# VisionDepth/VisionDepth3D

Hardware: AMD Instinct MI355X
Metric: stereo-pairs/sec end-to-end (depth+warp+fill+mux) (higher is better)
Workload: dtype f32; 1 GPU; 4k-dav2b-dibr; frame=3840x2160, format=Half-SBS, depth_model=depth-anything-v2-base, depth_net_dtype=float32 (the reference's precision), pixel_overlap=True, pixel_streams=2, clip_frames_all_ranks=32, params=render_cli.py defaults + dof_strength 2.0, dense DOF order (parity mode)

## Files before the change

### visiondepth3d_amd/csrc/vd3d_attn.hip

```cpp
#include "vd3d_dev.h"
#include "vd3d_kernels.h"
#include "vd3d_x3.h"

#include <mutex>

#define AT_D 64
#define AT_BQ 256
#define AT_BK 64
#define AT_NT 512
#define AT_NTERM(MODE) ((MODE) == 0 ? 3 : 2)
#define AT_TILE(MODE) (4 * AT_NTERM(MODE) * 2 * 64 * 16)
#define AT_STAGE(MODE) (2 * AT_TILE(MODE))
#define AT_NSTAGE 3
#define AT_LDS(MODE) (AT_NSTAGE * AT_STAGE(MODE))
#define AT_QBLK(MODE) (4 * AT_NTERM(MODE) * 2 * 32)
#define AT_QKV_SCALE 16.0f
#define AT_P_SCALE 1024.0f
#define AT_OP 272

struct vd_at_args {
  int B, H, T;
  int nq32, nkv, nqb;
  float c;
};

template <int MODE>
__global__ __launch_bounds__(256) void k_attn_x3_prep(const float* __restrict__ qkv, vd_at_args a, uint4* __restrict__ Qimg, uint4* __restrict__ Kimg,
                                                      uint4* __restrict__ Vimg) {
  constexpr int NTERM = AT_NTERM(MODE);
  const int which = blockIdx.z, bh = blockIdx.y, b = bh / a.H, h = bh - b * a.H;
  const int t_id = blockIdx.x * 256 + threadIdx.x;
  const size_t tok_stride = (size_t)3 * a.H * AT_D;
  float v[8];
  uint4* dst;
  if (which < 2) {
    const int rows = which == 0 ? a.nq32 * 32 : a.nkv * 64;
    const int t = t_id >> 3, c = t_id & 7;
    if (t >= rows) return;
    if (t < a.T) {
      const float* src = qkv + ((size_t)b * a.T + t) * tok_stride + (size_t)which * a.H * AT_D + h * AT_D + c * 8;
      const float4 lo = *reinterpret_cast<const float4*>(src), hi = *reinterpret_cast<const float4*>(src + 4);
      v[0] = lo.x; v[1] = lo.y; v[2] = lo.z; v[3] = lo.w; v[4] = hi.x; v[5] = hi.y; v[6] = hi.z; v[7] = hi.w;
    } else {
#pragma unroll
      for (int e = 0; e < 8; ++e) v[e] = 0.f;
    }
    const int ks = c >> 1, kh = c & 1;
    if (which == 0) dst = Qimg + ((size_t)bh * a.nq32 + (t >> 5)) * AT_QBLK(MODE) + (size_t)((ks * NTERM) * 2 + kh) * 32 + (t & 31);
    else dst = Kimg + ((size_t)bh * a.nkv + (t >> 6)) * (AT_TILE(MODE) / 16) + (size_t)((ks * NTERM) * 2 + kh) * 64 + (t & 63);
    x3_s8 o[NTERM];
    x3_split8_m<MODE>(v, AT_QKV_SCALE, o);
    const int ts = which == 0 ? 2 * 32 : 2 * 64;
#pragma unroll
    for (int t3 = 0; t3 < NTERM; ++t3) dst[(size_t)t3 * ts] = __builtin_bit_cast(uint4, o[t3]);
  } else {
    const int d = t_id & 63, kh = (t_id >> 6) & 1, ks = (t_id >> 7) & 3, tile = t_id >> 9;
    if (tile >= a.nkv) return;
    const int m = ks >> 1, j = ks & 1;
#pragma unroll
    for (int e = 0; e < 8; ++e) {
      const int kv = tile * 64 + 32 * m + (e & 3) + 8 * (2 * j + (e >> 2)) + 4 * kh;
      v[e] = kv < a.T ? qkv[((size_t)b * a.T + kv) * tok_stride + (size_t)2 * a.H * AT_D + h * AT_D + d] : 0.f;
    }
    x3_s8 o[NTERM];
    x3_split8_m<MODE>(v, AT_QKV_SCALE, o);
    dst = Vimg + ((size_t)bh * a.nkv + tile) * (AT_TILE(MODE) / 16) + (size_t)((ks * NTERM) * 2 + kh) * 64 + d;
#pragma unroll
    for (int t3 = 0; t3 < NTERM; ++t3) dst[(size_t)t3 * 128] = __builtin_bit_cast(uint4, o[t3]);
  }
}

#define AT_MM1(ACC0, AF0, ACC1, AF1, BF, ta, tb)                                               \
  ACC0 = x3_mfma<MODE>(AF0[ta], BF[tb], ACC0);                                                 \
  ACC1 = x3_mfma<MODE>(AF1[ta], BF[tb], ACC1);
#define AT_MM6(ACC0, AF0, ACC1, AF1, BF)                                                       \
  if (MODE == 0) { AT_MM1(ACC0, AF0, ACC1, AF1, BF, NTERM - 1, 0) AT_MM1(ACC0, AF0, ACC1, AF1, BF, 1, 1) AT_MM1(ACC0, AF0, ACC1, AF1, BF, 0, NTERM - 1) }                               \
  AT_MM1(ACC0, AF0, ACC1, AF1, BF, 1, 0) AT_MM1(ACC0, AF0, ACC1, AF1, BF, 0, 1) AT_MM1(ACC0, AF0, ACC1, AF1, BF, 0, 0)

template <int MODE>
__global__ __launch_bounds__(AT_NT) void k_attn_bf16x3(const uint4* __restrict__ Qimg, const uint4* __restrict__ Kimg, const uint4* __restrict__ Vimg,
                                                       float* __restrict__ out, vd_at_args a) {
  constexpr int NTERM = AT_NTERM(MODE), TILE = AT_TILE(MODE), STAGE = AT_STAGE(MODE), NP = TILE / (AT_NT * 16);
  extern __shared__ __attribute__((aligned(16))) uint8_t at_lds[];
  int bh, qb;
  {
    const int wg = blockIdx.x, x = wg & 7, idx = wg >> 3;
    const int g = idx / a.nqb;
    qb = idx - g * a.nqb;
    bh = g * 8 + x;
    if (bh >= a.B * a.H) return;
  }
  const int tid = threadIdx.x, lane = tid & 63, wave = __builtin_amdgcn_readfirstlane(tid >> 6);
  const int li = lane & 31, kh = lane >> 5;
  const int q0 = qb * AT_BQ + wave * 32;
  const int wave_base = (tid & ~63) * 16;

  x3_s8 qf[4][NTERM];
  {
    const int blk = min(q0 >> 5, a.nq32 - 1);
    const uint4* qp = Qimg + ((size_t)bh * a.nq32 + blk) * AT_QBLK(MODE) + kh * 32 + li;
#pragma unroll
    for (int ks = 0; ks < 4; ++ks)
#pragma unroll
      for (int t = 0; t < NTERM; ++t) qf[ks][t] = __builtin_bit_cast(x3_s8, qp[(ks * NTERM + t) * 64]);
  }
  const uint4* kimg = Kimg + (size_t)bh * a.nkv * (TILE / 16) + tid;
  const uint4* vimg = Vimg + (size_t)bh * a.nkv * (TILE / 16) + tid;
  auto dma = [&](int tile, int buf, int piece) {
    const int op = piece / 3, pp = piece - 3 * op;
    if (pp >= NP) return;
    const uint4* src = (op == 0 ? kimg : vimg) + (size_t)tile * (TILE / 16) + pp * AT_NT;
    uint8_t* dst = at_lds + buf * STAGE + op * TILE + pp * (AT_NT * 16) + wave_base;
    __builtin_amdgcn_global_load_lds((x3_glb_vp)src, (x3_lds_vp)dst, 16, 0, 0);
  };

  x3_f16 oacc[2];
#pragma unroll
  for (int dm = 0; dm < 2; ++dm)
#pragma unroll
    for (int r = 0; r < 16; ++r) oacc[dm][r] = 0.f;
  float m_run = -INFINITY, l_half = 0.f;

  const int last_tile = a.nkv - 1;
  auto tile_c = [&](int t) { return t < last_tile ? t : last_tile; };
#pragma unroll
  for (int p = 0; p < 6; ++p) dma(0, 0, p);
#pragma unroll
  for (int p = 0; p < 3; ++p) dma(tile_c(1), 1, p);
#pragma unroll
  for (int p = 3; p < 6; ++p) dma(tile_c(1), 1, p);
#pragma unroll
  for (int p = 0; p < 3; ++p) dma(tile_c(2), 2, p);
  if (NP == 3) asm volatile("s_waitcnt vmcnt(6)" ::: "memory"); else asm volatile("s_waitcnt vmcnt(4)" ::: "memory");
  __builtin_amdgcn_s_barrier();

  const int frag_off = (kh * 64 + li) * 16;
  auto st_step = [&](const uint8_t* sk, int ks, x3_f16 (&sa)[2]) {
    x3_s8 kf[2][NTERM];
#pragma unroll
    for (int m = 0; m < 2; ++m)
#pragma unroll
      for (int t = 0; t < NTERM; ++t) kf[m][t] = *reinterpret_cast<const x3_s8*>(sk + frag_off + ((ks * NTERM + t) * 2) * 1024 + m * 512);
    AT_MM6(sa[0], kf[0], sa[1], kf[1], qf[ks])
  };
#define AT_CHUNK_HINT(n)                                           \
  __builtin_amdgcn_sched_group_barrier(0x100, 6, 0);               \
  _Pragma("unroll") for (int i_ = 0; i_ < 12; ++i_) {              \
    __builtin_amdgcn_sched_group_barrier(0x008, 1, 0);             \
    __builtin_amdgcn_sched_group_barrier(0x002, n, 0);             \
  }                                                                \
  __builtin_amdgcn_sched_barrier(0);

  x3_f16 sacc[2];
#pragma unroll
  for (int m = 0; m < 2; ++m)
#pragma unroll
    for (int r = 0; r < 16; ++r) sacc[m][r] = 0.f;
#pragma unroll
  for (int ks = 0; ks < 4; ++ks) st_step(at_lds, ks, sacc);
  asm volatile("s_waitcnt lgkmcnt(0)" ::: "memory");
  __builtin_amdgcn_s_barrier();

  int cur = 0;
  for (int it = 0; it < a.nkv; ++it) {
    const int s1 = cur == 2 ? 0 : cur + 1, s2 = cur >= 1 ? cur - 1 : 2;
    const uint8_t* sk1 = at_lds + s1 * STAGE;
    const uint8_t* sv = at_lds + cur * STAGE + TILE;
    float z[2][16];
#pragma unroll
    for (int m = 0; m < 2; ++m)
#pragma unroll
      for (int r = 0; r < 16; ++r) z[m][r] = sacc[m][r] * a.c;
    if ((it + 1) * AT_BK > a.T) {
#pragma unroll
      for (int m = 0; m < 2; ++m)
#pragma unroll
        for (int r = 0; r < 16; ++r)
          if (it * AT_BK + 32 * m + (r & 3) + 8 * (r >> 2) + 4 * kh >= a.T) z[m][r] = -INFINITY;
    }
    x3_f16 sn[2];
#pragma unroll
    for (int m = 0; m < 2; ++m)
#pragma unroll
      for (int r = 0; r < 16; ++r) sn[m][r] = 0.f;
    dma(tile_c(it + 3), cur, 0);
    __builtin_amdgcn_sched_barrier(0);
    st_step(sk1, 0, sn);
    float mx = -INFINITY;
#pragma unroll
    for (int m = 0; m < 2; ++m)
#pragma unroll
      for (int r = 0; r < 16; ++r) mx = fmaxf(mx, z[m][r]);
    mx = fmaxf(mx, __shfl_xor(mx, 32, 64));
    const float m_new = fmaxf(m_run, mx);
    const float alpha = __builtin_amdgcn_exp2f(m_run - m_new);
    m_run = m_new;
    AT_CHUNK_HINT(2)
    float ps = 0.f;
#pragma unroll
    for (int m = 0; m < 2; ++m) {
      dma(tile_c(it + 3), cur, 1 + m);
      __builtin_amdgcn_sched_barrier(0);
      st_step(sk1, 1 + m, sn);
#pragma unroll
      for (int r = 0; r < 16; ++r) { z[m][r] = __builtin_amdgcn_exp2f(z[m][r] - m_new); ps += z[m][r]; }
      AT_CHUNK_HINT(4)
    }
    dma(tile_c(it + 2), s2, 3);
    __builtin_amdgcn_sched_barrier(0);
    st_step(sk1, 3, sn);
    l_half = l_half * alpha + ps;
#pragma unroll
    for (int dm = 0; dm < 2; ++dm)
#pragma unroll
      for (int r = 0; r < 16; ++r) oacc[dm][r] *= alpha;
    x3_s8 pf[2][NTERM];
    x3_split8_m<MODE>(&z[0][0], AT_P_SCALE, pf[0]);
    AT_CHUNK_HINT(7)
#pragma unroll
    for (int ks = 0; ks < 4; ++ks) {
      if (ks < 2) { dma(tile_c(it + 2), s2, 4 + ks); __builtin_amdgcn_sched_barrier(0); }
      if (ks < 3) x3_split8_m<MODE>(&z[(ks + 1) >> 1][8 * ((ks + 1) & 1)], AT_P_SCALE, pf[(ks + 1) & 1]);
      x3_s8 vf[2][NTERM];
#pragma unroll
      for (int dm = 0; dm < 2; ++dm)
#pragma unroll
        for (int t = 0; t < NTERM; ++t) vf[dm][t] = *reinterpret_cast<const x3_s8*>(sv + frag_off + ((ks * NTERM + t) * 2) * 1024 + dm * 512);
      AT_MM6(oacc[0], vf[0], oacc[1], vf[1], pf[ks & 1])
      AT_CHUNK_HINT(4)
    }
    if (NP == 3) asm volatile("s_waitcnt vmcnt(6) lgkmcnt(0)" ::: "memory"); else asm volatile("s_waitcnt vmcnt(4) lgkmcnt(0)" ::: "memory");
    __builtin_amdgcn_s_barrier();
#pragma unroll
    for (int m = 0; m < 2; ++m) sacc[m] = sn[m];
    cur = s1;
  }
#undef AT_CHUNK_HINT
  asm volatile("s_waitcnt vmcnt(0)" ::: "memory");
  __builtin_amdgcn_s_barrier();

  const float l_tot = l_half + __shfl_xor(l_half, 32, 64);
  const float inv = MODE == 1 ? 1.0f / (l_tot * (AT_P_SCALE * AT_QKV_SCALE)) : 1.0f / l_tot;
  uint8_t* ow = at_lds + wave * (32 * AT_OP);
#pragma unroll
  for (int dm = 0; dm < 2; ++dm)
#pragma unroll
    for (int g = 0; g < 4; ++g) {
      const float4 v4 = {oacc[dm][4 * g] * inv, oacc[dm][4 * g + 1] * inv, oacc[dm][4 * g + 2] * inv, oacc[dm][4 * g + 3] * inv};
      *reinterpret_cast<float4*>(ow + li * AT_OP + (32 * dm + 8 * g + 4 * kh) * 4) = v4;
    }
  asm volatile("s_waitcnt lgkmcnt(0)" ::: "memory");
  const int b = bh / a.H, h = bh - b * a.H;
#pragma unroll
  for (int i = 0; i < 8; ++i) {
    const int row = i * 4 + (lane >> 4), c4 = lane & 15;
    const int q = q0 + row;
    const float4 v4 = *reinterpret_cast<const float4*>(ow + row * AT_OP + c4 * 16);
    if (q < a.T) *reinterpret_cast<float4*>(out + (((size_t)b * a.T + q) * a.H + h) * AT_D + c4 * 4) = v4;
  }
}

#define AF_TILE (AT_BK * AT_D * 4)
#define AF_STAGE (2 * AF_TILE)
#define AF_LDS(NS) ((NS) * AF_STAGE)
static_assert(2 * AF_LDS(2) <= 160 * 1024, "two 4-wave workgroups per CU");
VD_DEV void af_st(const uint8_t* __restrict__ sk, const float (&qf)[32], int li, int kh, x3_f16 (&s)[2]) {
  const int kswz = (li & 15) << 4;
#pragma unroll
  for (int m = 0; m < 2; ++m)
#pragma unroll
    for (int r = 0; r < 16; ++r) s[m][r] = 0.f;
#pragma unroll
  for (int g = 0; g < 8; ++g) {
    float4 kf[2];
#pragma unroll
    for (int m = 0; m < 2; ++m) kf[m] = *reinterpret_cast<const float4*>(sk + (32 * m + li) * 256 + (((8 * kh + g) << 4) ^ kswz));
#pragma unroll
    for (int m = 0; m < 2; ++m) s[m] = __builtin_amdgcn_mfma_f32_32x32x2f32(kf[m].x, qf[4 * g], s[m], 0, 0, 0);
#pragma unroll
    for (int m = 0; m < 2; ++m) s[m] = __builtin_amdgcn_mfma_f32_32x32x2f32(kf[m].y, qf[4 * g + 1], s[m], 0, 0, 0);
#pragma unroll
    for (int m = 0; m < 2; ++m) s[m] = __builtin_amdgcn_mfma_f32_32x32x2f32(kf[m].z, qf[4 * g + 2], s[m], 0, 0, 0);
#pragma unroll
    for (int m = 0; m < 2; ++m) s[m] = __builtin_amdgcn_mfma_f32_32x32x2f32(kf[m].w, qf[4 * g + 3], s[m], 0, 0, 0);
  }
}
VD_DEV void af_pv(const uint8_t* __restrict__ sv, const x3_f16 (&p)[2], int li, int kh, x3_f16 (&oacc)[2]) {
#pragma unroll
  for (int m = 0; m < 2; ++m)
#pragma unroll
    for (int r = 0; r < 16; ++r) {
      const float2 vv = *reinterpret_cast<const float2*>(sv + (32 * m + (r & 3) + 8 * (r >> 2) + 4 * kh) * 256 + li * 8);
      oacc[0] = __builtin_amdgcn_mfma_f32_32x32x2f32(vv.x, p[m][r], oacc[0], 0, 0, 0);
      oacc[1] = __builtin_amdgcn_mfma_f32_32x32x2f32(vv.y, p[m][r], oacc[1], 0, 0, 0);
    }
}

template <int NW, int NS>
__global__ __launch_bounds__(NW * 64, NW == 4 ? 2 : 1) void k_attn_f32(const float* __restrict__ qkv, float* __restrict__ out, vd_at_args a) {
  static_assert((NW == 8 && NS == 3) || (NW == 4 && NS == 2), "built forms");
  constexpr int NP = 16 / NW;
  extern __shared__ __attribute__((aligned(16))) uint8_t at_lds[];
  int bh, qb;
  {
    const int wg = blockIdx.x, x = wg & 7, idx = wg >> 3;
    const int g = idx / a.nqb;
    qb = idx - g * a.nqb;
    bh = g * 8 + x;
    if (bh >= a.B * a.H) return;
  }
  const int tid = threadIdx.x, lane = tid & 63, wave = __builtin_amdgcn_readfirstlane(tid >> 6);
  const int li = lane & 31, kh = lane >> 5;
  const int q0 = qb * (NW * 32) + wave * 32;
  const bool live = NW == 8 || q0 < a.T;
  const int b = bh / a.H, h = bh - b * a.H;
  const size_t tok_stride = (size_t)3 * a.H * AT_D;
  const float* base = qkv + (size_t)b * a.T * tok_stride + h * AT_D;

  const int drow = tid >> 4, dpos = tid & 15, kchunk = dpos ^ (drow & 15);
  auto dma = [&](int tile, int stage) {
    uint8_t* dst = at_lds + stage * AF_STAGE + wave * 1024;
#pragma unroll
    for (int p = 0; p < NP; ++p) {
      const int tok = min(tile * AT_BK + drow + 4 * NW * p, a.T - 1);
      const float* src = base + (size_t)tok * tok_stride + a.H * AT_D;
      __builtin_amdgcn_global_load_lds((x3_glb_vp)(src + kchunk * 4), (x3_lds_vp)(dst + p * (NW * 1024)), 16, 0, 0);
      __builtin_amdgcn_global_load_lds((x3_glb_vp)(src + a.H * AT_D + dpos * 4), (x3_lds_vp)(dst + AF_TILE + p * (NW * 1024)), 16, 0, 0);
    }
  };

  float qf[32];
  if (live) {
    const float4* qp = reinterpret_cast<const float4*>(base + (size_t)min(q0 + li, a.T - 1) * tok_stride + 32 * kh);
#pragma unroll
    for (int g = 0; g < 8; ++g) {
      const float4 v = qp[g];
      qf[4 * g] = v.x * a.c; qf[4 * g + 1] = v.y * a.c; qf[4 * g + 2] = v.z * a.c; qf[4 * g + 3] = v.w * a.c;
    }
  } else {
#pragma unroll
    for (int g = 0; g < 32; ++g) qf[g] = 0.f;
  }
  dma(0, 0);
  if (NS == 3 && a.nkv > 1) {
    dma(1, 1);
    asm volatile("s_waitcnt vmcnt(4)" ::: "memory");
  } else {
    asm volatile("s_waitcnt vmcnt(0)" ::: "memory");
  }
  __builtin_amdgcn_s_barrier();

  x3_f16 oacc[2];
#pragma unroll
  for (int dm = 0; dm < 2; ++dm)
#pragma unroll
    for (int r = 0; r < 16; ++r) oacc[dm][r] = 0.f;
  float m_run = -INFINITY, l_half = 0.f;
  int cur = 0;
  for (int it = 0; it < a.nkv; ++it) {
    const bool ahead = it + (NS - 1) < a.nkv;
    if (NS == 3) { if (ahead) dma(it + 2, cur == 0 ? 2 : cur - 1); }
    else { if (ahead) dma(it + 1, cur ^ 1); }
    const uint8_t* sk = at_lds + cur * AF_STAGE;
    const uint8_t* sv = sk + AF_TILE;
    if (live) {
      x3_f16 s[2];
      af_st(sk, qf, li, kh, s);
      if ((it + 1) * AT_BK > a.T) {
#pragma unroll
        for (int m = 0; m < 2; ++m)
#pragma unroll
          for (int r = 0; r < 16; ++r)
            if (it * AT_BK + 32 * m + (r & 3) + 8 * (r >> 2) + 4 * kh >= a.T) s[m][r] = -INFINITY;
      }
      float mx = s[0][0];
#pragma unroll
      for (int m = 0; m < 2; ++m)
#pragma unroll
        for (int r = 0; r < 16; ++r) mx = fmaxf(mx, s[m][r]);
      mx = fmaxf(mx, __shfl_xor(mx, 32, 64));
      const float m_new = fmaxf(m_run, mx);
      if (__any(m_new > m_run)) {
        const float alpha = __builtin_amdgcn_exp2f(m_run - m_new);
#pragma unroll
        for (int dm = 0; dm < 2; ++dm)
#pragma unroll
          for (int r = 0; r < 16; ++r) oacc[dm][r] *= alpha;
        l_half *= alpha;
        m_run = m_new;
      }
      float ps = 0.f;
#pragma unroll
      for (int m = 0; m < 2; ++m)
#pragma unroll
        for (int r = 0; r < 16; ++r) { s[m][r] = __builtin_amdgcn_exp2f(s[m][r] - m_run); ps += s[m][r]; }
      l_half += ps;
      af_pv(sv, s, li, kh, oacc);
    }
    if (NS == 3 && ahead) asm volatile("s_waitcnt vmcnt(4) lgkmcnt(0)" ::: "memory"); else asm volatile("s_waitcnt vmcnt(0) lgkmcnt(0)" ::: "memory");
    __builtin_amdgcn_s_barrier();
    cur = NS == 3 ? (cur == 2 ? 0 : cur + 1) : cur ^ 1;
  }

  const float l_tot = l_half + __shfl_xor(l_half, 32, 64);
  const int q = q0 + li;
  if (q < a.T) {
    float* op = out + (((size_t)b * a.T + q) * a.H + h) * AT_D + 8 * kh;
#pragma unroll
    for (int g = 0; g < 4; ++g) {
      const float4 lo = {oacc[0][4 * g] / l_tot, oacc[1][4 * g] / l_tot, oacc[0][4 * g + 1] / l_tot, oacc[1][4 * g + 1] / l_tot};
      const float4 hi = {oacc[0][4 * g + 2] / l_tot, oacc[1][4 * g + 2] / l_tot, oacc[0][4 * g + 3] / l_tot, oacc[1][4 * g + 3] / l_tot};
      *reinterpret_cast<float4*>(op + 16 * g) = lo;
      *reinterpret_cast<float4*>(op + 16 * g + 4) = hi;
    }
  }
}

template <int NW, int NS>
static bool af_launch(hipStream_t s, const float* qkv, float* out, vd_at_args a) {
  static bool attr_set[64] = {};
  if (!vd_lds_optin({{reinterpret_cast<const void*>(k_attn_f32<NW, NS>), AF_LDS(NS)}}, attr_set)) return false;
  a.nqb = (a.T + NW * 32 - 1) / (NW * 32);
  const int groups = (a.B * a.H + 7) / 8;
  hipLaunchKernelGGL((k_attn_f32<NW, NS>), dim3((unsigned)(8 * groups * a.nqb)), dim3(NW * 64), AF_LDS(NS), s, qkv, out, a);
  return true;
}

bool vd_launch_attn_f32(hipStream_t s, const float* qkv, int B, int T, int H, int D, float scale, float* out, int form) {
  if (B < 1 || T < 1 || H < 1 || D != AT_D || (long long)B * H > 65535) return false;
  if (form != 0 && form != 4 && form != 8) return false;
  if ((reinterpret_cast<uintptr_t>(qkv) & 15) || (reinterpret_cast<uintptr_t>(out) & 15)) return false;
  vd_at_args a;
  a.B = B; a.H = H; a.T = T;
  a.nq32 = (T + 31) / 32; a.nkv = (T + AT_BK - 1) / AT_BK; a.nqb = 0;
  a.c = scale * 1.44269504088896340736f;
  if (form == 0) form = 8LL * ((B * H + 7) / 8) * ((T + AT_BQ - 1) / AT_BQ) >= 1024 ? 4 : 8;
  return form == 4 ? af_launch<4, 2>(s, qkv, out, a) : af_launch<8, 3>(s, qkv, out, a);
}

static bool at_mode_ok(int mode) { return mode == 0 || mode == 1; }
long long vd_attn_x3_workspace_bytes(int B, int T, int H, int D, int mode) {
  if (B < 1 || T < 1 || H < 1 || D != AT_D || !at_mode_ok(mode)) return -1;
  const long long nq32 = (T + 31) / 32, nkv = (T + AT_BK - 1) / AT_BK;
  const long long qblk = mode == 0 ? AT_QBLK(0) : AT_QBLK(1), tile = mode == 0 ? AT_TILE(0) : AT_TILE(1);
  return (long long)B * H * (nq32 * qblk * 16 + 2 * nkv * tile);
}

template <int MODE>
static bool at_launch(hipStream_t s, const float* qkv, int B, int T, int H, float scale, void* ws, float* out) {
  static bool attr_set[64] = {};
  if (!vd_lds_optin({{reinterpret_cast<const void*>(k_attn_bf16x3<MODE>), AT_LDS(MODE)}}, attr_set)) return false;
  vd_at_args a;
  a.B = B; a.H = H; a.T = T;
  a.nq32 = (T + 31) / 32; a.nkv = (T + AT_BK - 1) / AT_BK; a.nqb = (T + AT_BQ - 1) / AT_BQ;
  a.c = scale * 1.44269504088896340736f;
  if (MODE == 1) a.c *= 1.0f / (AT_QKV_SCALE * AT_QKV_SCALE);
  uint4* Qimg = reinterpret_cast<uint4*>(ws);
  uint4* Kimg = Qimg + (size_t)B * H * a.nq32 * AT_QBLK(MODE);
  uint4* Vimg = Kimg + (size_t)B * H * a.nkv * (AT_TILE(MODE) / 16);
  const int rows_max = a.nkv * 64 > a.nq32 * 32 ? a.nkv * 64 : a.nq32 * 32;
  hipLaunchKernelGGL(k_attn_x3_prep<MODE>, dim3((unsigned)((rows_max * 8 + 255) / 256), (unsigned)(B * H), 3), dim3(256), 0, s, qkv, a, Qimg, Kimg, Vimg);
  const int groups = (B * H + 7) / 8;
  hipLaunchKernelGGL(k_attn_bf16x3<MODE>, dim3((unsigned)(8 * groups * a.nqb)), dim3(AT_NT), AT_LDS(MODE), s, Qimg, Kimg, Vimg, out, a);
  return true;
}

bool vd_launch_attn_x3(hipStream_t s, const float* qkv, int B, int T, int H, int D, float scale, void* ws, float* out, int mode) {
  if (vd_attn_x3_workspace_bytes(B, T, H, D, mode) < 0) return false;
  if ((reinterpret_cast<uintptr_t>(qkv) & 15) || (reinterpret_cast<uintptr_t>(ws) & 15) || (reinterpret_cast<uintptr_t>(out) & 15)) return false;
  if ((long long)B * H > 65535) return false;
  return mode == 0 ? at_launch<0>(s, qkv, B, T, H, scale, ws, out) : at_launch<1>(s, qkv, B, T, H, scale, ws, out);
}
```

Before: 144.8 stereo-pairs/s.

## Unroll attention KV loop by ring depth with constant LDS offsets and tail specialization

Unrolls the f32 flash-attention KV loop by the number of pipeline stages so LDS stage offsets become compile-time immediates, and precomputes per-lane K/V LDS pointers once. Full tiles use a DMA path with scalar base plus a hoisted vector offset instead of recomputing clamped token addresses. A last tile with at most 32 valid keys is specialized to skip half the QK^T and PV MFMAs. The cross-half max reduction uses permlane32_swap instead of a shuffle. This adds code size and register pressure in exchange for less address arithmetic and less wasted tail work.

```diff
diff --git a/visiondepth3d_amd/csrc/vd3d_attn.hip b/visiondepth3d_amd/csrc/vd3d_attn.hip
--- a/visiondepth3d_amd/csrc/vd3d_attn.hip
+++ b/visiondepth3d_amd/csrc/vd3d_attn.hip
@@ -264,36 +264,39 @@
 #define AF_STAGE (2 * AF_TILE)
 #define AF_LDS(NS) ((NS) * AF_STAGE)
 static_assert(2 * AF_LDS(2) <= 160 * 1024, "two 4-wave workgroups per CU");
-VD_DEV void af_st(const uint8_t* __restrict__ sk, const float (&qf)[32], int li, int kh, x3_f16 (&s)[2]) {
-  const int kswz = (li & 15) << 4;
+static_assert(AF_LDS(2) == 65536 && AF_LDS(3) == 98304, "the rings' dynamic LDS; the two-stage ring ends at byte 65 535, the reach of a DS instruction's offset field");
+template <int N> struct af_ic { static constexpr int value = N; };
+template <int NM, int G>
+VD_DEV void af_st_g(const uint8_t* __restrict__ kp, int stage, const float (&qf)[32], x3_f16 (&s)[2]) {
+  float4 kf[NM];
+#pragma unroll
+  for (int m = 0; m < NM; ++m) kf[m] = *reinterpret_cast<const float4*>(kp + stage * AF_STAGE + 32 * 256 * m);
+#pragma unroll
+  for (int m = 0; m < NM; ++m) s[m] = __builtin_amdgcn_mfma_f32_32x32x2f32(kf[m].x, qf[4 * G], s[m], 0, 0, 0);
+#pragma unroll
+  for (int m = 0; m < NM; ++m) s[m] = __builtin_amdgcn_mfma_f32_32x32x2f32(kf[m].y, qf[4 * G + 1], s[m], 0, 0, 0);
+#pragma unroll
+  for (int m = 0; m < NM; ++m) s[m] = __builtin_amdgcn_mfma_f32_32x32x2f32(kf[m].z, qf[4 * G + 2], s[m], 0, 0, 0);
+#pragma unroll
+  for (int m = 0; m < NM; ++m) s[m] = __builtin_amdgcn_mfma_f32_32x32x2f32(kf[m].w, qf[4 * G + 3], s[m], 0, 0, 0);
+}
+template <int NM>
+VD_DEV void af_st(const uint8_t* const (&kp)[8], int stage, const float (&qf)[32], x3_f16 (&s)[2]) {
 #pragma unroll
   for (int m = 0; m < 2; ++m)
 #pragma unroll
-    for (int r = 0; r < 16; ++r) s[m][r] = 0.f;
-#pragma unroll
-  for (int g = 0; g < 8; ++g) {
-    float4 kf[2];
-#pragma unroll
-    for (int m = 0; m < 2; ++m) kf[m] = *reinterpret_cast<const float4*>(sk + (32 * m + li) * 256 + (((8 * kh + g) << 4) ^ kswz));
-#pragma unroll
-    for (int m = 0; m < 2; ++m) s[m] = __builtin_amdgcn_mfma_f32_32x32x2f32(kf[m].x, qf[4 * g], s[m], 0, 0, 0);
-#pragma unroll
-    for (int m = 0; m < 2; ++m) s[m] = __builtin_amdgcn_mfma_f32_32x32x2f32(kf[m].y, qf[4 * g + 1], s[m], 0, 0, 0);
-#pragma unroll
-    for (int m = 0; m < 2; ++m) s[m] = __builtin_amdgcn_mfma_f32_32x32x2f32(kf[m].z, qf[4 * g + 2], s[m], 0, 0, 0);
-#pragma unroll
-    for (int m = 0; m < 2; ++m) s[m] = __builtin_amdgcn_mfma_f32_32x32x2f32(kf[m].w, qf[4 * g + 3], s[m], 0, 0, 0);
-  }
-}
-VD_DEV void af_pv(const uint8_t* __restrict__ sv, const x3_f16 (&p)[2], int li, int kh, x3_f16 (&oacc)[2]) {
-#pragma unroll
-  for (int m = 0; m < 2; ++m)
-#pragma unroll
-    for (int r = 0; r < 16; ++r) {
-      const float2 vv = *reinterpret_cast<const float2*>(sv + (32 * m + (r & 3) + 8 * (r >> 2) + 4 * kh) * 256 + li * 8);
-      oacc[0] = __builtin_amdgcn_mfma_f32_32x32x2f32(vv.x, p[m][r], oacc[0], 0, 0, 0);
-      oacc[1] = __builtin_amdgcn_mfma_f32_32x32x2f32(vv.y, p[m][r], oacc[1], 0, 0, 0);
-    }
+    for (int r = 0; r < 16; ++r) s[m][r] = m < NM ? 0.f : -INFINITY;
+  af_st_g<NM, 0>(kp[0], stage, qf, s); af_st_g<NM, 1>(kp[1], stage, qf, s); af_st_g<NM, 2>(kp[2], stage, qf, s); af_st_g<NM, 3>(kp[3], stage, qf, s);
+  af_st_g<NM, 4>(kp[4], stage, qf, s); af_st_g<NM, 5>(kp[5], stage, qf, s); af_st_g<NM, 6>(kp[6], stage, qf, s); af_st_g<NM, 7>(kp[7], stage, qf, s);
+}
+template <int M>
+VD_DEV void af_pv(const uint8_t* __restrict__ sv, const x3_f16 (&p)[2], uint32_t va, x3_f16 (&oacc)[2]) {
+#pragma unroll
+  for (int r = 0; r < 16; ++r) {
+    const float2 vv = *reinterpret_cast<const float2*>(sv + va + (32 * M + (r & 3) + 8 * (r >> 2)) * 256);
+    oacc[0] = __builtin_amdgcn_mfma_f32_32x32x2f32(vv.x, p[M][r], oacc[0], 0, 0, 0);
+    oacc[1] = __builtin_amdgcn_mfma_f32_32x32x2f32(vv.y, p[M][r], oacc[1], 0, 0, 0);
+  }
 }
 
 template <int NW, int NS>
@@ -318,16 +321,36 @@
   const float* base = qkv + (size_t)b * a.T * tok_stride + h * AT_D;
 
   const int drow = tid >> 4, dpos = tid & 15, kchunk = dpos ^ (drow & 15);
+  const uint32_t tok_bytes = 3u * 4u * AT_D * (uint32_t)a.H;
+  const uint32_t koff = (uint32_t)drow * tok_bytes + (uint32_t)kchunk * 16u, voff = (uint32_t)drow * tok_bytes + (uint32_t)dpos * 16u;
+  const uint64_t kbase = reinterpret_cast<uint64_t>(base + a.H * AT_D), vbase = reinterpret_cast<uint64_t>(base + 2 * a.H * AT_D);
   auto dma = [&](int tile, int stage) {
     uint8_t* dst = at_lds + stage * AF_STAGE + wave * 1024;
-#pragma unroll
-    for (int p = 0; p < NP; ++p) {
-      const int tok = min(tile * AT_BK + drow + 4 * NW * p, a.T - 1);
-      const float* src = base + (size_t)tok * tok_stride + a.H * AT_D;
-      __builtin_amdgcn_global_load_lds((x3_glb_vp)(src + kchunk * 4), (x3_lds_vp)(dst + p * (NW * 1024)), 16, 0, 0);
-      __builtin_amdgcn_global_load_lds((x3_glb_vp)(src + a.H * AT_D + dpos * 4), (x3_lds_vp)(dst + AF_TILE + p * (NW * 1024)), 16, 0, 0);
+    if ((tile + 1) * AT_BK <= a.T) {
+      uint32_t ko = koff, vo = voff;
+      asm("" : "+v"(ko), "+v"(vo));
+#pragma unroll
+      for (int p = 0; p < NP; ++p) {
+        const uint64_t row0 = (uint64_t)(tile * AT_BK + 4 * NW * p) * tok_bytes;
+        uint64_t ks = kbase + row0, vs = vbase + row0;
+        asm("" : "+s"(ks), "+s"(vs));
+        __builtin_amdgcn_global_load_lds((x3_glb_vp)(ks + ko), (x3_lds_vp)(dst + p * (NW * 1024)), 16, 0, 0);
+        __builtin_amdgcn_global_load_lds((x3_glb_vp)(vs + vo), (x3_lds_vp)(dst + AF_TILE + p * (NW * 1024)), 16, 0, 0);
+      }
+    } else {
+#pragma unroll
+      for (int p = 0; p < NP; ++p) {
+        const int tok = min(tile * AT_BK + drow + 4 * NW * p, a.T - 1);
+        const float* src = base + (size_t)tok * tok_stride + a.H * AT_D;
+        __builtin_amdgcn_global_load_lds((x3_glb_vp)(src + kchunk * 4), (x3_lds_vp)(dst + p * (NW * 1024)), 16, 0, 0);
+        __builtin_amdgcn_global_load_lds((x3_glb_vp)(src + a.H * AT_D + dpos * 4), (x3_lds_vp)(dst + AF_TILE + p * (NW * 1024)), 16, 0, 0);
+      }
     }
   };
+  const uint8_t* kp[8];
+#pragma unroll
+  for (int g = 0; g < 8; ++g) kp[g] = at_lds + (li * 256 + (((8 * kh + g) << 4) ^ ((li & 15) << 4)));
+  const uint32_t va = (uint32_t)(kh * 1024 + li * 8);
 
   float qf[32];
   if (live) {
@@ -356,19 +379,17 @@
 #pragma unroll
     for (int r = 0; r < 16; ++r) oacc[dm][r] = 0.f;
   float m_run = -INFINITY, l_half = 0.f;
-  int cur = 0;
-  for (int it = 0; it < a.nkv; ++it) {
+  auto tile = [&](int it, int stage, auto nm) __attribute__((always_inline)) {
+    constexpr int NM = decltype(nm)::value;
     const bool ahead = it + (NS - 1) < a.nkv;
-    if (NS == 3) { if (ahead) dma(it + 2, cur == 0 ? 2 : cur - 1); }
-    else { if (ahead) dma(it + 1, cur ^ 1); }
-    const uint8_t* sk = at_lds + cur * AF_STAGE;
-    const uint8_t* sv = sk + AF_TILE;
+    if (ahead) dma(it + (NS - 1), (stage + NS - 1) % NS);
+    const uint8_t* sv = at_lds + stage * AF_STAGE + AF_TILE;
     if (live) {
       x3_f16 s[2];
-      af_st(sk, qf, li, kh, s);
+      af_st<NM>(kp, stage, qf, s);
       if ((it + 1) * AT_BK > a.T) {
 #pragma unroll
-        for (int m = 0; m < 2; ++m)
+        for (int m = 0; m < NM; ++m)
 #pragma unroll
           for (int r = 0; r < 16; ++r)
             if (it * AT_BK + 32 * m + (r & 3) + 8 * (r >> 2) + 4 * kh >= a.T) s[m][r] = -INFINITY;
@@ -378,7 +399,10 @@
       for (int m = 0; m < 2; ++m)
 #pragma unroll
         for (int r = 0; r < 16; ++r) mx = fmaxf(mx, s[m][r]);
-      mx = fmaxf(mx, __shfl_xor(mx, 32, 64));
+      {
+        const auto sw = __builtin_amdgcn_permlane32_swap(__float_as_uint(mx), __float_as_uint(mx), false, false);
+        mx = fmaxf(__uint_as_float(sw[0]), __uint_as_float(sw[1]));
+      }
       const float m_new = fmaxf(m_run, mx);
       if (__any(m_new > m_run)) {
         const float alpha = __builtin_amdgcn_exp2f(m_run - m_new);
@@ -395,12 +419,21 @@
 #pragma unroll
         for (int r = 0; r < 16; ++r) { s[m][r] = __builtin_amdgcn_exp2f(s[m][r] - m_run); ps += s[m][r]; }
       l_half += ps;
-      af_pv(sv, s, li, kh, oacc);
+      af_pv<0>(sv, s, va, oacc);
+      if (NM == 2) af_pv<1>(sv, s, va, oacc);
     }
     if (NS == 3 && ahead) asm volatile("s_waitcnt vmcnt(4) lgkmcnt(0)" ::: "memory"); else asm volatile("s_waitcnt vmcnt(0) lgkmcnt(0)" ::: "memory");
     __builtin_amdgcn_s_barrier();
-    cur = NS == 3 ? (cur == 2 ? 0 : cur + 1) : cur ^ 1;
-  }
+  };
+  const int nfull = (a.nkv - 1) * AT_BK + 32 >= a.T ? a.nkv - 1 : a.nkv;
+  for (int it0 = 0; it0 < nfull; it0 += NS) {
+#pragma unroll
+    for (int u = 0; u < NS; ++u) {
+      if (it0 + u >= nfull) break;
+      tile(it0 + u, u, af_ic<2>());
+    }
+  }
+  if (nfull < a.nkv) tile(nfull, nfull % NS, af_ic<1>());
 
   const float l_tot = l_half + __shfl_xor(l_half, 32, 64);
   const int q = q0 + li;
```

Result: faster. 146.5 stereo-pairs/s (median of 6 runs) (+1.2%).
